# RupertLuo/Valley

Measured on NVIDIA H100. Metric: generated tokens/s (8-frame video requests: ViT-L/14 encode + pool/project + LLaMA prefill + 256 greedy tokens per sequence), higher is better.
Workload: dtype bf16

## Files before the change

### valley_b200/csrc/api.cu

```cuda
#include <cuda_runtime.h>
#include <cuda.h>

#include <algorithm>
#include <atomic>
#include <cmath>
#include <cstdarg>
#include <cstdio>
#include <cstdlib>
#include <cstring>
#include <map>
#include <memory>
#include <mutex>
#include <string>
#include <type_traits>
#include <utility>
#include <vector>

#include "../../include/valley_b200.h"
#include "attention_tc.cuh"
#include "common.cuh"
#include "gemm_tc.cuh"
#include "simt_kernels.cuh"
#include "decode_kernels.cuh"
#include "decode_mega.cuh"
// ... 967 lines not shown
    GemmParams p = {};
    p.M = T * NP; p.N = 2 * H; p.K = H; p.out = KV; p.ldo = 2 * H; p.bias = w.in_b + H;
    TRY(launch_gemm<EPI_BIAS>(c, pick_bn_m(c, p.N, p.M), Xp, H, w.in_w + (size_t)H * H, H, p, st));
    p = {};
    p.M = NP; p.N = H; p.K = H; p.out = Q; p.ldo = H; p.bias = w.in_b;
    TRY(launch_gemm<EPI_BIAS>(c, pick_bn_m(c, p.N, p.M), Xlast, H, w.in_w, H, p, st));
    TRY(launch(c, delta_attention_kernel, {dim3(NP), dim3(nhead * 32), 0, st}, Q, KV, att, T, NP, H, nhead));
    p = {};
    p.M = NP; p.N = H; p.K = H; p.out = X1; p.ldo = H; p.bias = w.out_b; p.residual = Xlast; p.ldr = H;
    TRY(launch_gemm<EPI_BIAS_RES_STATS>(c, pick_bn_m(c, p.N, p.M), att, H, w.out_w, H, p, st));
    TRY(launch(c, layernorm_rows_kernel, {dim3(NP), dim3(256), 0, st}, X1, w.n1_g, w.n1_b, X1, H, 1e-5f));
    p = {};
    p.M = NP; p.N = w.ffn; p.K = H; p.out = F1; p.ldo = w.ffn; p.bias = w.l1_b;
    TRY(launch_gemm<EPI_BIAS>(c, pick_bn_m(c, p.N, p.M), X1, H, w.l1_w, H, p, st));
    TRY(launch(c, relu_inplace_kernel, {dim3(c->num_sms), dim3(256), 0, st}, F1, (long long)NP * w.ffn / 8));
    p = {};
    p.M = NP; p.N = H; p.K = w.ffn; p.out = X2; p.ldo = H; p.bias = w.l2_b; p.residual = X1; p.ldr = H;
    TRY(launch_gemm<EPI_BIAS_RES_STATS>(c, pick_bn_m(c, p.N, p.M), F1, w.ffn, w.l2_w, w.ffn, p, st));
    TRY(launch(c, layernorm_rows_kernel, {dim3(NP), dim3(256), 0, st}, X2, w.n2_g, w.n2_b, X2, H, 1e-5f));
    TRY(launch(c, delta_finish_kernel, two_per_sm, P, X2, vis, T, tokens, H));
  }
  return VLY_OK;
}

extern "C" int vly_pool_project(vly_ctx* c, const void* feats, int n_videos, int T, void* vis_rows, void* stream) {
  if (!c || !feats || !vis_rows || n_videos <= 0 || T <= 0) return fail(VLY_ERR_INVALID, "vly_pool_project: bad argument");
  std::lock_guard<std::mutex> lk(c->mu);
  if (!c->finalized || !c->proj_w) return fail(VLY_ERR_STATE, "vly_pool_project: mm_projector not loaded");
  CK(cudaSetDevice(c->cfg.device));
  cudaStream_t st = (cudaStream_t)stream;
  const vly_config& g = c->cfg;
  const int D = g.vit_hidden, tokens = (g.vit_image / g.vit_patch) * (g.vit_image / g.vit_patch) + 1;
  const int rows = tokens - 1 + T;
  if (g.patch_pooling_method == VLY_POOL_MAX || g.patch_pooling_method == VLY_POOL_TEMPORAL_TRANSFORMER)
    return pool_project_after(c, (const bf16*)feats, n_videos, T, (bf16*)vis_rows, st);
  TRY(ensure(c->w_pool, (size_t)n_videos * rows * D * 2));
  if (g.patch_pooling_method == VLY_POOL_TEMPORAL_IMPORTANCE) {
    if (!c->pool_U) return fail(VLY_ERR_STATE, "vly_pool_project: model.pooling_layer.weight not loaded");
    TRY(ensure(c->w_score, (size_t)n_videos * T * 4));
    TRY(launch(c, importance_score_kernel, {dim3(T, n_videos), dim3(256), 0, st}, (const bf16*)feats, c->pool_U, (float*)c->w_score.p, T,
               tokens, D));
    TRY(launch(c, weighted_pool_kernel, {dim3(c->num_sms * 4), dim3(256), 0, st}, (const bf16*)feats, (const float*)c->w_score.p,
               (bf16*)c->w_pool.p, n_videos, T, tokens, D));
  } else {
    TRY(launch(c, temporal_pool_kernel, {dim3(c->num_sms * 4), dim3(256), 0, st}, (const bf16*)feats, (bf16*)c->w_pool.p, n_videos, T,
               tokens, D));
  }
  GemmParams p = {};
  p.M = n_videos * rows; p.N = g.hidden_size; p.K = D;
  p.out = vis_rows; p.ldo = g.hidden_size; p.bias = c->proj_b;
  return launch_gemm<EPI_BIAS>(c, pick_bn(p.N), (bf16*)c->w_pool.p, D, c->proj_w, D, p, st);
}

extern "C" int vly_embed_splice(vly_ctx* c, const int64_t* ids, const int32_t* src_map, const int32_t* img_idx, const void* vis_rows,
                                int rows_per_img, int B, int S, void* out, void* stream) {
  if (!c || !ids || !out || B <= 0 || S <= 0) return fail(VLY_ERR_INVALID, "vly_embed_splice: bad argument");
  if (src_map && (!img_idx || !vis_rows)) return fail(VLY_ERR_INVALID, "vly_embed_splice: src_map given without img_idx / vis_rows");
  std::lock_guard<std::mutex> lk(c->mu);
  if (!c->finalized || !c->has_llm) return fail(VLY_ERR_STATE, "vly_embed_splice: LLM weights not loaded");
  CK(cudaSetDevice(c->cfg.device));
  return launch(c, embed_splice_kernel, {dim3(B * S), dim3(128), 0, (cudaStream_t)stream}, (const long long*)ids, src_map, img_idx, c->embed,
                (const bf16*)vis_rows, rows_per_img, (bf16*)out, nullptr, 0, S, c->cfg.hidden_size, c->cfg.vocab_size);
}

static void mega_smem_layout(const vly_config& g, int bmax, size_t* x_bytes, size_t* misc) {
  const bool tc = bmax > 1;
  const int kmax = g.intermediate_size > g.hidden_size ? g.intermediate_size : g.hidden_size;
  const size_t xs_stride_b = tc ? (size_t)(((kmax * 2 + 127) & ~127) + MegaCfg::PAD_TC) : (size_t)kmax * 2;
  *x_bytes = ((size_t)bmax * xs_stride_b + 127) & ~size_t(127);
  const int nv = (tc ? MegaCfg::ROWS_TC : MegaCfg::ROWS) * bmax;
  *misc = (2 * MegaCfg::MAX_STAGES + 2 * MegaCfg::RED_SLOTS + 2) * 8 + (size_t)MegaCfg::RED_SLOTS * 16 * nv * 4 + (3 + 16) * bmax * 4 + 256;
}
static const size_t kMegaSmem = 226 * 1024;
static const int kMegaDbgCounters = 1024 * 8;

struct DecodeSettings {
  int stage_kb = 0;
  int rows = 0;
  int inflight_kb = 100;
  int stages = 0;
  int inflight = 0;
  int attn_ikeys = 0;
  int l2_hint = 1;
  bool dbg = false;
};
static DecodeSettings read_decode_settings() {
  auto num = [](const char* name, int unset) {
    const char* v = getenv(name);
    return v ? atoi(v) : unset;
  };
  DecodeSettings s;
  s.stage_kb = num("VLY_MEGA_STAGE_KB", 0);
  s.rows = num("VLY_MEGA_ROWS", 0);
  s.inflight_kb = num("VLY_MEGA_INFLIGHT_KB", 100);
  s.stages = num("VLY_MEGA_STAGES", 0);
  s.inflight = num("VLY_MEGA_INFLIGHT", 0);
  const int ik = num("VLY_ATTN_IKEYS", 0);
  s.attn_ikeys = (ik >= 16 && ik <= 256 && ik % 16 == 0) ? ik : 0;
  const char* hint = getenv("VLY_MEGA_L2_HINT");
  s.l2_hint = (hint && *hint) ? atoi(hint) != 0 : 1;
  s.dbg = getenv("VLY_MEGA_DBG") != nullptr;
  return s;
}

static void pick_phase_geometry(const DecodeSettings& s, int bmax, size_t ring_budget, int N, int K, int num_sms, int* rows_out,
                                int* kc_out) {
  const bool tc = bmax > 1;
  const int max_rows = tc ? MegaCfg::ROWS_TC : MegaCfg::ROWS;
  const int pad = tc ? MegaCfg::PAD_TC : 0, gran = tc ? 64 : 8;
  size_t target = s.stage_kb > 0 ? (size_t)s.stage_kb * 1024 : (tc ? 33 * 1024 + 512 : 41 * 1024);
  if (target > ring_budget / 2) target = ring_budget / 2;
  if (target < 8 * 1024) target = 8 * 1024;
  auto kc_for = [&](int rows) {
    const int cap = (int)((target / rows - pad) / 2);
    const int ns = cdiv(K, cap > gran ? cap : gran);
    int kc = cdiv(cdiv(K, ns), gran) * gran;
    return kc > K ? cdiv(K, gran) * gran : kc;
  };
  int rows = max_rows;
  if (s.rows > 0) rows = s.rows > max_rows ? max_rows : s.rows;
  else {
    if (kc_for(rows) * 2 < 3072 && K * 2 >= 3072) rows = max_rows / 2;
    if (rows == max_rows && !tc) {
      const long long load_full = (long long)cdiv(cdiv(N, max_rows), num_sms) * max_rows;
      const long long load_half = (long long)cdiv(cdiv(N, max_rows / 2), num_sms) * (max_rows / 2);
      if (load_half * 100 < load_full * 97) rows = max_rows / 2;
    }
  }
  *rows_out = rows;
  *kc_out = kc_for(rows);
}

static int plan_decode_mega(vly_ctx* c, vly_kv* kv, const DecodeSettings& s) {
  const vly_config& g = c->cfg;
  const int B = kv->B, H = g.hidden_size, nH = g.num_attention_heads, I = g.intermediate_size, V = g.vocab_size;
  const int bmax = bmax_of(B);
  const int pad = bmax > 1 ? MegaCfg::PAD_TC : 0;
  size_t x_bytes, misc;
  mega_smem_layout(g, bmax, &x_bytes, &misc);
  const size_t ring_budget = kMegaSmem > x_bytes + misc ? kMegaSmem - x_bytes - misc : 0;
  std::vector<PhaseDesc> ph;
  int stage_bytes = 0;
  auto add = [&](PhaseDesc d) {
    d.rows = d.kc = 0;
    if (d.type != PH_ATTN) {
      pick_phase_geometry(s, bmax, ring_budget, d.N, d.K, c->num_sms, &d.rows, &d.kc);
      const int sb = d.rows * (d.kc * 2 + pad);
      if (sb > stage_bytes) stage_bytes = sb;
    }
    ph.push_back(d);
  };
  for (int l = 0; l < g.num_hidden_layers; ++l) {
    const LlamaLayerW& w = c->layers[l];
    PhaseDesc d = {};
    d.layer = l; d.kcache = kv->k_layer(l); d.vcache = kv->v_layer(l);
    d.type = PH_QKV; d.N = 3 * H; d.K = H; d.W = w.wqkv; d.x_in = kv->x; d.out = kv->q; add(d);
    d.type = PH_ATTN; d.N = 0; d.K = 0; d.W = nullptr; d.x_in = nullptr; d.out = kv->attn; add(d);
    d.type = PH_OPROJ; d.N = H; d.K = H; d.W = w.wo; d.x_in = kv->attn; d.out = kv->x; add(d);
    d.type = PH_GATEUP; d.N = 2 * I; d.K = H; d.W = w.wgu; d.x_in = kv->x; d.out = kv->hb; add(d);
    d.type = PH_DOWN; d.N = H; d.K = I; d.W = w.wdown; d.x_in = kv->hb; d.out = kv->x; add(d);
  }
  {
    PhaseDesc d = {};
    d.type = PH_LOGITS; d.N = V; d.K = H; d.W = c->lm_head; d.x_in = kv->x; d.out = nullptr; add(d);
  }
  stage_bytes = (stage_bytes + 127) & ~127;
  for (PhaseDesc& q : ph) {
    if (q.type == PH_ATTN) continue;
    const int sb = q.rows * (q.kc * 2 + pad);
    q.inflight = (s.inflight_kb * 1024 + sb / 2) / sb;
    if (q.inflight < 2) q.inflight = 2;
  }
  int n_stages = (int)(((long long)kMegaSmem - (long long)x_bytes - (long long)misc) / (long long)stage_bytes);
  if (n_stages > MegaCfg::MAX_STAGES) n_stages = MegaCfg::MAX_STAGES;
  const int cap = s.stages > 0 ? s.stages : 4;
  if (n_stages > cap) n_stages = cap;
  if (n_stages < 2)
    return fail(VLY_ERR_INVALID, "vly_kv_create: activations (B=%d, K=%d) leave no room for the weight ring (%d stages, at least 2 needed)",
                B, std::max(I, H), n_stages);
  if (s.dbg) {
    fprintf(stderr, "[vly] decode ring: B=%d x=%zu B, ring budget %zu B, slot %d B, %d slots fit, %d used;", B, x_bytes, ring_budget,
            stage_bytes, (int)(ring_budget / stage_bytes), n_stages);
    for (int i = 0; i < 5 && i < (int)ph.size(); ++i)
      if (ph[i].type != PH_ATTN) fprintf(stderr, " type%d N=%d K=%d rows=%d kc=%d inflight=%d;", ph[i].type, ph[i].N, ph[i].K, ph[i].rows, ph[i].kc, ph[i].inflight);
    fprintf(stderr, " logits rows=%d kc=%d\n", ph.back().rows, ph.back().kc);
    TRY(kv->dbg.alloc(kMegaDbgCounters * sizeof(long long)));
  }
  TRY(kv->d_phases.alloc(ph.size() * sizeof(PhaseDesc)));
  CK(cudaMemcpy(kv->d_phases, ph.data(), ph.size() * sizeof(PhaseDesc), cudaMemcpyHostToDevice));

  StepParams& p = kv->mega;
  p = {};
  p.phases = kv->d_phases; p.n_phases = (int)ph.size();
  p.B = B; p.H = H; p.nH = nH; p.Smax = kv->Smax; p.V = V;
  p.Kmax = std::max(I, H);
  p.eps = g.rms_norm_eps; p.scale_log2e = 0.08838834764831845f * 1.4426950408889634f;
  p.rope = c->rope; p.seq_len = kv->d_len; p.step = kv->d_step; p.embed = c->embed; p.tokens_in = kv->cur_tokens;
  p.x = kv->x; p.q = kv->q; p.attn = kv->attn;
  p.part_o = kv->part_o; p.part_ml = kv->part_ml; p.attn_counters = kv->counters; p.nsplit = kv->nsplit;
  p.key_bits = kv->key_bits; p.mask_words = kv->mask_words();
  p.logits = kv->logits; p.part_val = kv->part_val; p.part_idx = kv->part_idx;
  p.next_tokens = kv->cur_tokens; p.out_tokens = kv->gen_tokens; p.out_stride = kv->Smax;
  p.sample = kv->d_sample;
  p.grid_counter = kv->counters + (size_t)B * nH + 1;
  p.grid_epoch = p.grid_counter + 1;
  p.n_grid_syncs = p.n_phases + 1;
  p.attn_ikeys = s.attn_ikeys;
  p.n_stages = n_stages;
  p.stage_bytes = stage_bytes;
  p.n_inflight = s.inflight > 0 ? s.inflight : n_stages;
  if (p.n_inflight > n_stages) p.n_inflight = n_stages;
  p.l2_hint = s.l2_hint;
  p.dbg = kv->dbg;
  kv->mega_smem = (size_t)n_stages * stage_bytes + x_bytes + misc;
  return VLY_OK;
}

extern "C" int vly_kv_create(vly_ctx* c, int batch, int max_seq, vly_kv** out) {
  if (!c || !out || batch <= 0 || max_seq <= 0) return fail(VLY_ERR_INVALID, "vly_kv_create: bad argument");
  if (!c->finalized || !c->has_llm) return fail(VLY_ERR_STATE, "vly_kv_create: LLM weights not finalised");
  if (max_seq > c->cfg.max_position_embeddings) return fail(VLY_ERR_INVALID, "vly_kv_create: max_seq %d > max_position_embeddings %d", max_seq, c->cfg.max_position_embeddings);
  CK(cudaSetDevice(c->cfg.device));
  const vly_config& g = c->cfg;
  auto kv = std::make_unique<vly_kv>();
  kv->ctx = c;
  kv->B = batch;
  kv->Smax = (max_seq + 127) / 128 * 128;
  const int H = g.hidden_size, nH = g.num_attention_heads, I = g.intermediate_size, V = g.vocab_size, L = g.num_hidden_layers;
  const size_t cache_elems = (size_t)L * kv->layer_stride();
  TRY(kv->cache.alloc(cache_elems * 2));
  CK(cudaMemset(kv->cache, 0, cache_elems * 2));
  kv->nsplit = kv->Smax / MegaCfg::ATTN_KEYS_MIN;
  TRY(kv->d_len.alloc(8));
  TRY(kv->h_len.alloc(sizeof(int), true));
  CK(cudaEventCreateWithFlags(&kv->len_event, cudaEventDisableTiming));
  kv->d_step = kv->d_len + 1;
  CK(cudaMemset(kv->d_len, 0, 8));
  const size_t act_rows = batch < 8 ? 8 : batch;
  TRY(kv->x.alloc(act_rows * H * 2));
  TRY(kv->q.alloc(act_rows * H * 2));
  TRY(kv->attn.alloc(act_rows * H * 2));
  TRY(kv->hb.alloc(act_rows * I * 2));
  CK(cudaMemset(kv->x, 0, act_rows * H * 2));
  CK(cudaMemset(kv->attn, 0, act_rows * H * 2));
  CK(cudaMemset(kv->hb, 0, act_rows * I * 2));
  TRY(kv->part_o.alloc((size_t)batch * nH * kv->nsplit * 128 * 4));
  TRY(kv->part_ml.alloc((size_t)batch * nH * kv->nsplit * sizeof(float2)));
  TRY(kv->counters.alloc(((size_t)batch * nH + 4) * 4));
  CK(cudaMemset(kv->counters, 0, ((size_t)batch * nH + 4) * 4));
  TRY(kv->part_val.alloc((size_t)batch * c->num_sms * 4));
  TRY(kv->part_idx.alloc((size_t)batch * c->num_sms * 4));
  TRY(kv->logits.alloc((size_t)batch * V * 4));
  TRY(kv->cur_tokens.alloc((size_t)batch * 8));
  TRY(kv->gen_tokens.alloc((size_t)batch * kv->Smax * 8));
  TRY(kv->d_sample.alloc(sizeof(SampleState)));
  {
    const SampleState s0 = {};
    CK(cudaMemcpy(kv->d_sample, &s0, sizeof(s0), cudaMemcpyHostToDevice));
  }
  TRY(kv->key_bits.alloc((size_t)batch * kv->mask_words() * 4));
  CK(cudaMemset(kv->key_bits, 0xff, (size_t)batch * kv->mask_words() * 4));
  if (batch <= 4) TRY(plan_decode_mega(c, kv.get(), read_decode_settings()));
  *out = kv.release();
  return VLY_OK;
}

extern "C" int vly_kv_decode_kernel(vly_kv* kv, char* name, int cap) {
  if (!kv || !name || cap <= 0) return fail(VLY_ERR_INVALID, "vly_kv_decode_kernel: bad argument");
  if (kv->B <= 4) snprintf(name, (size_t)cap, "decode_step_kernel<%d>", bmax_of(kv->B));
  else snprintf(name, (size_t)cap, "per-op TMA-ring decode kernels");
  return VLY_OK;
}

extern "C" void vly_kv_destroy(vly_kv* kv) {
  if (!kv) return;
  cudaSetDevice(kv->ctx->cfg.device);
  delete kv;
}

extern "C" int vly_kv_seq_len(vly_kv* kv, int* out) {
  if (!kv || !out) return fail(VLY_ERR_INVALID, "null");
  TRY(sync_len(kv));
  *out = kv->host_len;
  return VLY_OK;
}

extern "C" int vly_kv_reset(vly_kv* kv, void* stream) {
  if (!kv) return fail(VLY_ERR_INVALID, "null");
  CK(cudaSetDevice(kv->ctx->cfg.device));
  kv->host_len = 0;
  kv->len_dirty = false;
  CK(cudaMemsetAsync(kv->d_len, 0, 8, (cudaStream_t)stream));
  if (kv->masked) {
    CK(cudaMemsetAsync(kv->key_bits, 0xff, (size_t)kv->B * kv->mask_words() * 4, (cudaStream_t)stream));
    kv->masked = false;
// ... 753 lines not shown
```

### valley_b200/csrc/common.cuh

```cuda
#pragma once
#include <cuda_runtime.h>
#include <cuda_bf16.h>
#include <cuda_fp16.h>
#include <cuda.h>
#include <stdint.h>

#define VLY_DEVINL __device__ __forceinline__

namespace vly {

VLY_DEVINL uint32_t smem_u32(const void* p) { return static_cast<uint32_t>(__cvta_generic_to_shared(p)); }

VLY_DEVINL uint32_t pack_bf16x2(float lo, float hi) {
  __nv_bfloat162 v = __floats2bfloat162_rn(lo, hi);
  return *reinterpret_cast<uint32_t*>(&v);
}
VLY_DEVINL float bf16_lo(uint32_t v) { return __uint_as_float(v << 16); }
VLY_DEVINL float bf16_hi(uint32_t v) { return __uint_as_float(v & 0xffff0000u); }
VLY_DEVINL float bf16_round(float x) { return __bfloat162float(__float2bfloat16_rn(x)); }

VLY_DEVINL void mbar_init(uint64_t* bar, uint32_t count) {
  asm volatile("mbarrier.init.shared::cta.b64 [%0], %1;\n" ::"r"(smem_u32(bar)), "r"(count));
}
VLY_DEVINL void fence_barrier_init() { asm volatile("fence.mbarrier_init.release.cluster;\n" ::: "memory"); }

VLY_DEVINL void mbar_expect_tx(uint64_t* bar, uint32_t bytes) {
  asm volatile("mbarrier.arrive.expect_tx.shared::cta.b64 _, [%0], %1;\n" ::"r"(smem_u32(bar)), "r"(bytes) : "memory");
}
VLY_DEVINL void mbar_arrive(uint64_t* bar) {
  asm volatile("mbarrier.arrive.shared::cta.b64 _, [%0];\n" ::"r"(smem_u32(bar)) : "memory");
}
VLY_DEVINL bool mbar_try_wait(uint64_t* bar, uint32_t parity) {
  uint32_t ok;
  asm volatile(
      "{\n\t.reg .pred P;\n\t"
      "mbarrier.try_wait.parity.shared::cta.b64 P, [%1], %2;\n\t"
      "selp.b32 %0, 1, 0, P;\n\t}\n"
      : "=r"(ok)
      : "r"(smem_u32(bar)), "r"(parity)
      : "memory");
  return ok != 0;
}
VLY_DEVINL void mbar_wait(uint64_t* bar, uint32_t parity) {
  while (!mbar_try_wait(bar, parity)) {
  }
}

VLY_DEVINL void tma_prefetch_desc(const CUtensorMap* m) {
  asm volatile("prefetch.tensormap [%0];\n" ::"l"(reinterpret_cast<uint64_t>(m)) : "memory");
}
VLY_DEVINL void tma_load_2d(void* smem_dst, const CUtensorMap* m, uint64_t* bar, int c0, int c1) {
  asm volatile(
      "cp.async.bulk.tensor.2d.shared::cluster.global.mbarrier::complete_tx::bytes [%0], [%1, {%3, %4}], [%2];\n" ::"r"(
          smem_u32(smem_dst)),
      "l"(reinterpret_cast<uint64_t>(m)), "r"(smem_u32(bar)), "r"(c0), "r"(c1)
      : "memory");
}
VLY_DEVINL void tma_load_3d(void* smem_dst, const CUtensorMap* m, uint64_t* bar, int c0, int c1, int c2) {
  asm volatile(
      "cp.async.bulk.tensor.3d.shared::cluster.global.mbarrier::complete_tx::bytes [%0], [%1, {%3, %4, %5}], [%2];\n" ::"r"(
          smem_u32(smem_dst)),
      "l"(reinterpret_cast<uint64_t>(m)), "r"(smem_u32(bar)), "r"(c0), "r"(c1), "r"(c2)
      : "memory");
}

VLY_DEVINL void bulk_load_1d(void* smem_dst, const void* gsrc, uint32_t bytes, uint64_t* bar) {
  asm volatile("cp.async.bulk.shared::cluster.global.mbarrier::complete_tx::bytes [%0], [%1], %2, [%3];\n" ::"r"(smem_u32(smem_dst)),
               "l"(gsrc), "r"(bytes), "r"(smem_u32(bar))
               : "memory");
}
VLY_DEVINL void bulk_load_1d_hint(void* smem_dst, const void* gsrc, uint32_t bytes, uint64_t* bar, uint64_t policy) {
  asm volatile("cp.async.bulk.shared::cluster.global.mbarrier::complete_tx::bytes.L2::cache_hint [%0], [%1], %2, [%3], %4;\n" ::"r"(
                   smem_u32(smem_dst)),
               "l"(gsrc), "r"(bytes), "r"(smem_u32(bar)), "l"(policy)
               : "memory");
}
VLY_DEVINL uint64_t l2_policy_evict_first() {
  uint64_t p;
  asm volatile("createpolicy.fractional.L2::evict_first.b64 %0, 1.0;\n" : "=l"(p));
  return p;
}
VLY_DEVINL void pdl_wait() { asm volatile("griddepcontrol.wait;\n" ::: "memory"); }
VLY_DEVINL void pdl_launch_dependents() { asm volatile("griddepcontrol.launch_dependents;\n" ::: "memory"); }

VLY_DEVINL uint64_t make_smem_desc_sw128(uint32_t smem_addr, uint32_t lbo_bytes, uint32_t sbo_bytes) {
  uint64_t d = 0;
  d |= uint64_t((smem_addr >> 4) & 0x3FFF);
  d |= uint64_t((lbo_bytes >> 4) & 0x3FFF) << 16;
  d |= uint64_t((sbo_bytes >> 4) & 0x3FFF) << 32;
  d |= uint64_t(1) << 62;
  return d;
}

VLY_DEVINL float fast_exp2(float x) {
  float y;
  asm("ex2.approx.ftz.f32 %0, %1;" : "=f"(y) : "f"(x));
  return y;
}

VLY_DEVINL float warp_sum(float v) {
#pragma unroll
  for (int o = 16; o > 0; o >>= 1) v += __shfl_xor_sync(0xffffffffu, v, o);
  return v;
}
VLY_DEVINL float warp_max(float v) {
#pragma unroll
  for (int o = 16; o > 0; o >>= 1) v = fmaxf(v, __shfl_xor_sync(0xffffffffu, v, o));
  return v;
}
VLY_DEVINL void warp_argmax(float& v, int& i) {
#pragma unroll
  for (int o = 16; o > 0; o >>= 1) {
    const float ov = __shfl_xor_sync(0xffffffffu, v, o);
    const int oi = __shfl_xor_sync(0xffffffffu, i, o);
    if (ov > v || (ov == v && oi < i)) { v = ov; i = oi; }
  }
}

}
```

### valley_b200/csrc/decode_mega.cuh

```cuda
#pragma once
#include "common.cuh"
#include "simt_kernels.cuh"
#include "decode_kernels.cuh"
#include "sampling.cuh"

namespace vly {

enum PhaseType : int { PH_QKV = 0, PH_ATTN = 1, PH_OPROJ = 2, PH_GATEUP = 3, PH_DOWN = 4, PH_LOGITS = 5 };

struct PhaseDesc {
  int type, N, K, layer;
  int rows, kc;
  int inflight;
  const __nv_bfloat16* W;
  const __nv_bfloat16* x_in;
  __nv_bfloat16* out;
  __nv_bfloat16* kcache;
  __nv_bfloat16* vcache;
};

struct StepParams {
  const PhaseDesc* phases;
  int n_phases;
  int B, H, nH, Smax, V, Kmax;
  float eps, scale_log2e;
  const float2* rope;
  int* seq_len;
  int* step;
  const __nv_bfloat16* embed;
  const long long* tokens_in;
  __nv_bfloat16* x;
  const __nv_bfloat16* q;
  __nv_bfloat16* attn;
  float* part_o;
  float2* part_ml;
  unsigned int* attn_counters;
  int nsplit;
  const uint32_t* key_bits;
  int mask_words;
  float* logits;
  float* part_val;
  int* part_idx;
  long long* next_tokens;
  long long* out_tokens;
  int out_stride;
  SampleState* sample;
  unsigned int* grid_counter;
  unsigned int* grid_epoch;
  int n_grid_syncs;
  int attn_ikeys;
  int n_stages;
  int stage_bytes;
  int n_inflight;
  int l2_hint;
  long long* dbg;
  int select;
};

struct MegaCfg {
  static constexpr int ROWS = 4;
  static constexpr int ROWS_TC = 8;
  static constexpr int PAD_TC = 64;
  static constexpr int CONSUMERS = 512, THREADS = 576;
  static constexpr int RED_SLOTS = 4;
  static constexpr int MAX_STAGES = 8;
  static constexpr int ATTN_KEYS_MIN = 16;
};

VLY_DEVINL uint4 ldcg_v4(const void* p) {
  uint4 r;
  asm volatile("ld.global.cg.v4.u32 {%0, %1, %2, %3}, [%4];\n" : "=r"(r.x), "=r"(r.y), "=r"(r.z), "=r"(r.w) : "l"(p) : "memory");
  return r;
}
VLY_DEVINL float ldcg_bf16(const __nv_bfloat16* p) {
  unsigned short v;
  asm volatile("ld.global.cg.u16 %0, [%1];\n" : "=h"(v) : "l"(p) : "memory");
  return __uint_as_float((uint32_t)v << 16);
}
VLY_DEVINL void mma_m16n8k16_bf16(float (&d)[4], uint32_t a0, uint32_t a1, uint32_t a2, uint32_t a3, uint32_t b0, uint32_t b1) {
  asm volatile("mma.sync.aligned.m16n8k16.row.col.f32.bf16.bf16.f32 {%0,%1,%2,%3}, {%4,%5,%6,%7}, {%8,%9}, {%0,%1,%2,%3};\n"
               : "+f"(d[0]), "+f"(d[1]), "+f"(d[2]), "+f"(d[3])
               : "r"(a0), "r"(a1), "r"(a2), "r"(a3), "r"(b0), "r"(b1));
}

VLY_DEVINL uint32_t ld_acquire_u32(const unsigned int* p) {
  uint32_t v;
  asm volatile("ld.acquire.gpu.global.u32 %0, [%1];\n" : "=r"(v) : "l"(p) : "memory");
  return v;
}
VLY_DEVINL void fence_proxy_async_global() { asm volatile("fence.proxy.async.global;\n" ::: "memory"); }

VLY_DEVINL void grid_sync_consumers(unsigned int* counter, unsigned int target, int ct) {
  asm volatile("bar.sync 2, 544;" ::: "memory");
  if (ct == 0) {
    asm volatile("red.release.gpu.global.add.u32 [%0], 1;\n" ::"l"(counter) : "memory");
    while ((int)(ld_acquire_u32(counter) - target) < 0) {
    }
  }
  asm volatile("bar.sync 2, 544;" ::: "memory");
}

VLY_DEVINL void mega_attention_phase(const StepParams& p, const PhaseDesc& d, const int cw, const int lane, const int pos) {
  const int len = pos + 1;
  const int n_warps = 16 * (int)gridDim.x;
  int ikeys = p.attn_ikeys;
  if (ikeys == 0) {
    if (p.B * p.nH * ((len + 15) >> 4) <= n_warps) ikeys = 16;
    else
      for (ikeys = 32; ikeys < 256; ikeys += 16)
        if (p.B * p.nH * ((len + ikeys - 1) / ikeys) <= n_warps + n_warps / 20) break;
  }
  const int n_act = (len + ikeys - 1) / ikeys;
  const int items = p.B * p.nH * n_act;
  const int hl = lane & 15, hw = lane >> 4;
  for (int it = cw * gridDim.x + blockIdx.x; it < items; it += gridDim.x * 16) {
    const int split = it % n_act, bh = it / n_act;
    const int b = bh / p.nH, h = bh - b * p.nH;
    const int k0 = split * ikeys, nk = min(len - k0, ikeys);
    const __nv_bfloat16* kb = d.kcache + ((size_t)bh * p.Smax + k0) * 128 + hl * 8;
    const __nv_bfloat16* vb = d.vcache + ((size_t)bh * p.Smax + k0) * 128 + hl * 8;
    const uint32_t* kbw = p.key_bits + (size_t)b * p.mask_words;
    float qf[8];
    {
      const uint4 w = ldcg_v4(p.q + (size_t)b * p.H + h * 128 + hl * 8);
      qf[0] = bf16_lo(w.x); qf[1] = bf16_hi(w.x); qf[2] = bf16_lo(w.y); qf[3] = bf16_hi(w.y);
      qf[4] = bf16_lo(w.z); qf[5] = bf16_hi(w.z); qf[6] = bf16_lo(w.w); qf[7] = bf16_hi(w.w);
    }
    float m_run = -INFINITY, l_run = 0.f;
    float o[8] = {0.f, 0.f, 0.f, 0.f, 0.f, 0.f, 0.f, 0.f};
#pragma unroll 1
    for (int kk0 = 0; kk0 < nk; kk0 += 16) {
      const uint32_t kbits = __ldg(kbw + ((k0 + kk0) >> 5)) >> ((k0 + kk0) & 31);
      uint4 kw[8], vw[8];
#pragma unroll
      for (int j = 0; j < 8; ++j) {
        const int key = kk0 + 2 * j + hw;
        const bool ok = key < nk;
        kw[j] = ok ? ldcg_v4(kb + (size_t)key * 128) : make_uint4(0, 0, 0, 0);
        vw[j] = ok ? ldcg_v4(vb + (size_t)key * 128) : make_uint4(0, 0, 0, 0);
      }
      float sc[8];
#pragma unroll
      for (int j = 0; j < 8; ++j) {
        const uint4 w = kw[j];
        sc[j] = qf[0] * bf16_lo(w.x) + qf[1] * bf16_hi(w.x) + qf[2] * bf16_lo(w.y) + qf[3] * bf16_hi(w.y) +
                qf[4] * bf16_lo(w.z) + qf[5] * bf16_hi(w.z) + qf[6] * bf16_lo(w.w) + qf[7] * bf16_hi(w.w);
      }

#pragma unroll
      for (int off = 8, n = 4; off >= 2; off >>= 1, n >>= 1) {
        const bool up = (hl & off) != 0;
#pragma unroll
        for (int i = 0; i < 4; ++i) {
          if (i < n) {
            const float send = up ? sc[i] : sc[i + n];
            const float keep = up ? sc[i + n] : sc[i];
            sc[i] = keep + __shfl_xor_sync(0xffffffffu, send, off);
          }
        }
      }
      sc[0] += __shfl_xor_sync(0xffffffffu, sc[0], 1);
      const int my_key = kk0 + 2 * (hl >> 1) + hw;
      const bool valid = my_key < nk && ((kbits >> (my_key - kk0)) & 1u);
      const float s_my = valid ? sc[0] * p.scale_log2e : -INFINITY;
      float mx = s_my;
      mx = fmaxf(mx, __shfl_xor_sync(0xffffffffu, mx, 2));
// ... 126 lines not shown
      const float ov = __shfl_xor_sync(kMask, bv, o);
      const int oi = __shfl_xor_sync(kMask, bi, o);
      if (ov > bv || (ov == bv && oi < bi)) { bv = ov; bi = oi; }
    }
    if (lane < BMAX && lane < p.B && bv > bestv[lane]) {
      bestv[lane] = bv;
      besti[lane] = bi;
    }
  } else {
    const float mine = t * rstd_s[b];
    const float other = __shfl_xor_sync(kMask, mine, BMAX);
    if ((r & 1) == 0 && ok && n + 1 < d.N) {
      float x0 = mine, x1 = other;
      if (d.type == PH_GATEUP) {
        const float gte = bf16_round(x0), up = bf16_round(x1);
        d.out[(size_t)b * (d.N >> 1) + (n >> 1)] = __float2bfloat16_rn(bf16_round(gte / (1.f + __expf(-gte))) * up);
      } else {
        const int which = n / p.H, nh = n - which * p.H, head = nh >> 7, cidx = nh & 127;
        if (which < 2) {
          const float a = x0 * pre0 - x1 * pre1, c2 = x1 * pre0 + x0 * pre1;
          x0 = a;
          x1 = c2;
        }
        __nv_bfloat16* dst;
        if (which == 0) dst = d.out + (size_t)b * p.H + nh;
        else dst = ((which == 1) ? d.kcache : d.vcache) + (((size_t)b * p.nH + head) * p.Smax + pos) * 128 + cidx;
        *reinterpret_cast<uint32_t*>(dst) = pack_bf16x2(x0, x1);
      }
    }
  }
}

VLY_DEVINL void mega_finish_step(const StepParams& p, const int cw, const int lane, const int ct) {
  if (cw < p.B) {
    const int b = cw;
    float bv = -INFINITY;
    int bi = 0x7fffffff;
    for (int g = lane; g < (int)gridDim.x; g += 32) {
      const float v = __ldcg(p.part_val + (size_t)b * gridDim.x + g);
      const int i = __ldcg(p.part_idx + (size_t)b * gridDim.x + g);
      if (v > bv || (v == bv && i < bi)) { bv = v; bi = i; }
    }
    warp_argmax(bv, bi);
    if (lane == 0) {
      const long long tok = p.select ? sample_finish_row(p.sample, b, bi) : bi;
      p.next_tokens[b] = tok;
      if (p.out_tokens != nullptr) p.out_tokens[(size_t)b * p.out_stride + *p.step] = tok;
    }
  }
  asm volatile("bar.sync 7, 512;" ::: "memory");
  if (ct == 0) {
    *p.step += 1;
    *p.seq_len += 1;
    *p.grid_epoch += 1;
    if (p.select) sample_close_step(p.sample, p.B, true);
    else p.sample->steps_valid += 1;
  }
}

template <int BMAX>
__global__ void __launch_bounds__(576, 1) decode_step_kernel(const StepParams p) {
  using M = MegaCfg;
  constexpr bool kTC = BMAX > 1;
  constexpr int ROWS = kTC ? M::ROWS_TC : M::ROWS;
  constexpr int NV = ROWS * BMAX;
  constexpr int PAD = kTC ? M::PAD_TC : 0;
  extern __shared__ uint8_t msm_raw[];
  uint8_t* msm = msm_raw + ((128u - (smem_u32(msm_raw) & 127u)) & 127u);
  uint8_t* ring = msm;
  __nv_bfloat16* xs = reinterpret_cast<__nv_bfloat16*>(ring + (size_t)p.n_stages * p.stage_bytes);
  const int xs_stride = kTC ? (((p.Kmax * 2 + 127) & ~127) + PAD) / 2 : p.Kmax;
  const size_t xs_bytes = ((size_t)BMAX * xs_stride * 2 + 127) & ~size_t(127);
  uint8_t* tail = reinterpret_cast<uint8_t*>(xs) + xs_bytes;
  uint64_t* full_bar = reinterpret_cast<uint64_t*>(tail);
  uint64_t* empty_bar = full_bar + M::MAX_STAGES;
  uint64_t* red_full = empty_bar + M::MAX_STAGES;
  uint64_t* red_empty = red_full + M::RED_SLOTS;
  uint64_t* x_bar = red_empty + M::RED_SLOTS;
  float* red = reinterpret_cast<float*>(x_bar + 2);
  float* rstd_s = red + M::RED_SLOTS * 16 * NV;
  float* bestv = rstd_s + BMAX;
  int* besti = reinterpret_cast<int*>(bestv + BMAX);
  float* wred = reinterpret_cast<float*>(besti + BMAX);

  const int tid = threadIdx.x, warp = tid >> 5, lane = tid & 31;
  if (p.sample->all_done) return;
  if (tid == 0) {
    for (int i = 0; i < p.n_stages; ++i) {
      mbar_init(&full_bar[i], 1);
      mbar_init(&empty_bar[i], 16);
    }
    for (int i = 0; i < M::RED_SLOTS; ++i) {
      mbar_init(&red_full[i], 16);
      mbar_init(&red_empty[i], 1);
    }
    mbar_init(x_bar, 1);
    fence_barrier_init();
  }
  __syncthreads();

  if (warp == 0) {
    if (lane == 0) {
      int st = 0;
      uint32_t ph = 0;
      int wst = 0, issued = 0, confirmed = 0;
      uint32_t wph = 0;
      long long* dbg_p = p.dbg != nullptr ? p.dbg + (size_t)blockIdx.x * 32 : nullptr;
      if (dbg_p != nullptr)
        for (int i = 26; i < 32; ++i) dbg_p[i] = 0;
      const bool hint = p.l2_hint != 0;
      const uint64_t pol_stream = l2_policy_evict_first();
      for (int pi = 0; pi < p.n_phases; ++pi) {
        const PhaseDesc d = p.phases[pi];
        if (d.type == PH_ATTN) continue;
        const int rows_u = d.rows, KCp = d.kc;
        const int row_stride = KCp * 2 + PAD;
        const int n_groups = (d.N + rows_u - 1) / rows_u;
        const int n_slices = (d.K + KCp - 1) / KCp;
        const int infl = min(d.inflight, p.n_inflight);
        long long t_blocked = 0;
        for (int g = blockIdx.x; g < n_groups; g += gridDim.x) {
          const int n0 = g * rows_u;
          const int rows = min(rows_u, d.N - n0);
          for (int s = 0; s < n_slices; ++s) {
            const int kc = min(KCp, d.K - s * KCp);
            const long long t_w = dbg_p != nullptr ? clock64() : 0;
            mbar_wait(&empty_bar[st], ph ^ 1);
            while (issued - confirmed >= infl) {
              mbar_wait(&full_bar[wst], wph);
              if (++wst == p.n_stages) { wst = 0; wph ^= 1; }
              ++confirmed;
            }
            if (dbg_p != nullptr) t_blocked += clock64() - t_w;
            ++issued;
            mbar_expect_tx(&full_bar[st], (uint32_t)rows * kc * 2);
            uint8_t* dst = ring + (size_t)st * p.stage_bytes;
            const __nv_bfloat16* src = d.W + (size_t)n0 * d.K + (size_t)s * KCp;
            if (PAD == 0 && kc == d.K) {
              if (hint) bulk_load_1d_hint(dst, src, (uint32_t)rows * kc * 2, &full_bar[st], pol_stream);
              else bulk_load_1d(dst, src, (uint32_t)rows * kc * 2, &full_bar[st]);
            } else if (hint) {
              for (int r = 0; r < rows; ++r)
                bulk_load_1d_hint(dst + r * row_stride, src + (size_t)r * d.K, (uint32_t)kc * 2, &full_bar[st], pol_stream);
            } else {
              for (int r = 0; r < rows; ++r) bulk_load_1d(dst + r * row_stride, src + (size_t)r * d.K, (uint32_t)kc * 2, &full_bar[st]);
            }
            if (++st == p.n_stages) { st = 0; ph ^= 1; }
          }
        }
        if (dbg_p != nullptr) dbg_p[26 + d.type] += t_blocked;
      }
    }
    return;
  }

  const bool is_fin = (warp == 17);
  const int ct = tid - 32;
  const int cw = warp - 1;
  const int pos = *p.seq_len;
  const bool samp_on = p.select && p.sample->enabled != 0;
  const float samp_it = p.sample->inv_temp;
  const uint32_t samp_k0 = p.sample->seed_lo, samp_k1 = p.sample->seed_hi;
  unsigned int sync_no = 0;
  const unsigned int sync_base = *p.grid_epoch * (unsigned int)p.n_grid_syncs * gridDim.x;
  long long t_sync = 0, t_stage = 0, t_loop = 0, t_attn = 0, t0 = clock64();
  long long* dbg_o = (p.dbg != nullptr && ct == 0) ? p.dbg + (size_t)blockIdx.x * 32 : nullptr;
  if (dbg_o != nullptr)
    for (int i = 8; i < 26; ++i) dbg_o[i] = 0;
  {
    if (!is_fin) {
      const int chunks = p.B * (p.H >> 3);
      for (int i = blockIdx.x * M::CONSUMERS + ct; i < chunks; i += gridDim.x * M::CONSUMERS) {
        const int b = i / (p.H >> 3), c = i % (p.H >> 3);
        long long id = p.tokens_in[b];
        id = id < 0 ? 0 : (id >= p.V ? p.V - 1 : id);
        *reinterpret_cast<uint4*>(p.x + (size_t)b * p.H + c * 8) = *reinterpret_cast<const uint4*>(p.embed + (size_t)id * p.H + c * 8);
      }
    } else if (lane < BMAX) {
      bestv[lane] = -INFINITY;
      besti[lane] = 0;
    }
    grid_sync_consumers(p.grid_counter, sync_base + (++sync_no) * gridDim.x, ct);
    t_sync += clock64() - t0;
  }

  int st = 0;
  uint32_t ph = 0, xph = 0;
  unsigned int unit_no = 0;
  for (int pi = 0; pi < p.n_phases; ++pi) {
    const PhaseDesc d = p.phases[pi];
    t0 = clock64();
    if (d.type == PH_ATTN) {
      if (!is_fin) mega_attention_phase(p, d, cw, lane, pos);
      t_attn += clock64() - t0;
      if (dbg_o != nullptr) dbg_o[8 + 3 * PH_ATTN + 1] += clock64() - t0;
    } else {
      const bool norm = (d.type == PH_QKV || d.type == PH_GATEUP || d.type == PH_LOGITS);
      const int rows_u = d.rows, KCp = d.kc;
      const int row_stride = KCp * 2 + PAD;
      if (!is_fin) {
        if (ct == 0) {
          fence_proxy_async_global();
          mbar_expect_tx(x_bar, (uint32_t)p.B * d.K * 2);
          for (int b = 0; b < p.B; ++b) bulk_load_1d(xs + (size_t)b * xs_stride, d.x_in + (size_t)b * d.K, (uint32_t)d.K * 2, x_bar);
        }
        mbar_wait(x_bar, xph);
        if (norm) {
          float sq[BMAX];
#pragma unroll
          for (int b = 0; b < BMAX; ++b) sq[b] = 0.f;
          const int chunks = d.K >> 3;
          for (int c = ct; c < chunks; c += M::CONSUMERS) {
#pragma unroll
            for (int b = 0; b < BMAX; ++b) {
              if (b < p.B) {
                const uint4 w = *reinterpret_cast<const uint4*>(xs + (size_t)b * xs_stride + c * 8);
                const uint32_t ww[4] = {w.x, w.y, w.z, w.w};
#pragma unroll
                for (int i = 0; i < 4; ++i) {
                  const float a = bf16_lo(ww[i]), bb = bf16_hi(ww[i]);
                  sq[b] += a * a + bb * bb;
                }
              }
            }
          }
#pragma unroll
          for (int b = 0; b < BMAX; ++b) {
            const float v = warp_sum(sq[b]);
            if (lane == 0) wred[cw * BMAX + b] = v;
          }
        }
      }
      xph ^= 1;
      if (norm) {
        asm volatile("bar.sync 2, 544;" ::: "memory");
        if (!is_fin && ct < BMAX) {
          float t = 0.f;
          for (int w = 0; w < 16; ++w) t += wred[w * BMAX + ct];
          rstd_s[ct] = rsqrtf(t / d.K + p.eps);
        }
        asm volatile("bar.sync 2, 544;" ::: "memory");
      }
      t_stage += clock64() - t0;
      if (dbg_o != nullptr) dbg_o[8 + 3 * d.type] += clock64() - t0;
      t0 = clock64();
      const int n_groups = (d.N + rows_u - 1) / rows_u;
      const int n_slices = (d.K + KCp - 1) / KCp;
      if (!is_fin) {
        for (int g = blockIdx.x; g < n_groups; g += gridDim.x, ++unit_no) {
          const int n0 = g * rows_u;
          const int rows = min(rows_u, d.N - n0);
          const int slot = unit_no & (M::RED_SLOTS - 1);
          const uint32_t round = (unit_no / M::RED_SLOTS) & 1;
          if constexpr (kTC) {
            const int gq = lane >> 2, tq = lane & 3;
            float dacc[4] = {0.f, 0.f, 0.f, 0.f}, dacc1[4] = {0.f, 0.f, 0.f, 0.f};
            const bool w_ok = gq < rows, x_ok = gq < p.B;
            for (int s = 0; s < n_slices; ++s) {
              const int kc = min(KCp, d.K - s * KCp);
              mbar_wait(&full_bar[st], ph);
              const uint8_t* wrow = ring + (size_t)st * p.stage_bytes + gq * row_stride;
              const __nv_bfloat16* xrow = xs + (size_t)gq * xs_stride + (size_t)s * KCp;
              const int nblk = kc >> 5, bpw = (nblk + 15) >> 4;
              const int kb0 = cw * bpw, kb1 = min(kb0 + bpw, nblk);
#pragma unroll 4
              for (int kb = kb0; kb < kb1; ++kb) {
                const int k = kb << 5;
                uint4 wb = make_uint4(0, 0, 0, 0), xa = make_uint4(0, 0, 0, 0);
                if (w_ok) wb = *reinterpret_cast<const uint4*>(wrow + (k + tq * 8) * 2);
                if (x_ok) xa = *reinterpret_cast<const uint4*>(xrow + k + tq * 8);
                mma_m16n8k16_bf16(dacc, xa.x, 0u, xa.y, 0u, wb.x, wb.y);
                mma_m16n8k16_bf16(dacc1, xa.z, 0u, xa.w, 0u, wb.z, wb.w);
              }
              __syncwarp();
              if (lane == 0) mbar_arrive(&empty_bar[st]);
              if (++st == p.n_stages) { st = 0; ph ^= 1; }
            }
            dacc[0] += dacc1[0];
            dacc[1] += dacc1[1];
            mbar_wait(&red_empty[slot], round ^ 1);
            if (gq < BMAX) {
              float* rp = red + (slot * 16 + cw) * NV;
              rp[(2 * tq) * BMAX + gq] = dacc[0];
              rp[(2 * tq + 1) * BMAX + gq] = dacc[1];
            }
            __syncwarp();
            if (lane == 0) mbar_arrive(&red_full[slot]);
            continue;
          }
          float acc[NV];
#pragma unroll
          for (int i = 0; i < NV; ++i) acc[i] = 0.f;
          for (int s = 0; s < n_slices; ++s) {
            const int kc = min(KCp, d.K - s * KCp);
            mbar_wait(&full_bar[st], ph);
            for (int c8 = ct * 8; c8 < kc; c8 += M::CONSUMERS * 8) {
              const uint8_t* src = ring + (size_t)st * p.stage_bytes + c8 * 2;
              float xf[BMAX][8];
#pragma unroll
              for (int b = 0; b < BMAX; ++b) {
                const uint4 xv = *reinterpret_cast<const uint4*>(xs + (size_t)b * xs_stride + (size_t)s * KCp + c8);
                xf[b][0] = bf16_lo(xv.x); xf[b][1] = bf16_hi(xv.x); xf[b][2] = bf16_lo(xv.y); xf[b][3] = bf16_hi(xv.y);
                xf[b][4] = bf16_lo(xv.z); xf[b][5] = bf16_hi(xv.z); xf[b][6] = bf16_lo(xv.w); xf[b][7] = bf16_hi(xv.w);
              }
#pragma unroll
              for (int r = 0; r < ROWS; ++r) {
                if (r < rows) {
                  const uint4 wv = *reinterpret_cast<const uint4*>(src + r * row_stride);
                  const float wf[8] = {bf16_lo(wv.x), bf16_hi(wv.x), bf16_lo(wv.y), bf16_hi(wv.y),
                                       bf16_lo(wv.z), bf16_hi(wv.z), bf16_lo(wv.w), bf16_hi(wv.w)};
#pragma unroll
                  for (int b = 0; b < BMAX; ++b)
#pragma unroll
                    for (int e = 0; e < 8; ++e) acc[r * BMAX + b] = fmaf(wf[e], xf[b][e], acc[r * BMAX + b]);
                }
              }
            }
            __syncwarp();
            if (lane == 0) mbar_arrive(&empty_bar[st]);
            if (++st == p.n_stages) { st = 0; ph ^= 1; }
          }
          warp_reduce_scatter<NV>(acc, lane);
          mbar_wait(&red_empty[slot], round ^ 1);
          if ((lane & (32 / NV - 1)) == 0) red[(slot * 16 + cw) * NV + lane / (32 / NV)] = acc[0];
          __syncwarp();
          if (lane == 0) mbar_arrive(&red_full[slot]);
        }
      } else {
        for (int g = blockIdx.x; g < n_groups; g += gridDim.x, ++unit_no) {
          const int n0 = g * rows_u;
          const int slot = unit_no & (M::RED_SLOTS - 1);
          const uint32_t round = (unit_no / M::RED_SLOTS) & 1;
          const int r = lane / BMAX, b = lane % BMAX, n = n0 + r;
          const bool ok = lane < NV && r < rows_u && b < p.B && n < d.N;
          float pre0 = 0.f, pre1 = 0.f;
          mega_epilogue_prefetch(p, d, ok, b, n, pos, pre0, pre1);
          mbar_wait(&red_full[slot], round);
          float t = 0.f;
          if (lane < NV) {
#pragma unroll
            for (int w = 0; w < 16; ++w) t += red[(slot * 16 + w) * NV + lane];
          }
          __syncwarp();
          if (lane == 0) mbar_arrive(&red_empty[slot]);
          if (lane < NV)
            mega_unit_epilogue<BMAX, NV>(p, d, lane, t, ok, r, b, n, pre0, pre1, pos, rstd_s, bestv, besti, samp_on, samp_it, samp_k0, samp_k1);
        }
      }
      t_loop += clock64() - t0;
      if (dbg_o != nullptr) dbg_o[8 + 3 * d.type + 1] += clock64() - t0;
    }
    t0 = clock64();
    if (pi == p.n_phases - 1 && is_fin && lane < p.B) {
      p.part_val[(size_t)lane * gridDim.x + blockIdx.x] = bestv[lane];
      p.part_idx[(size_t)lane * gridDim.x + blockIdx.x] = besti[lane];
    }
    grid_sync_consumers(p.grid_counter, sync_base + (++sync_no) * gridDim.x, ct);
    t_sync += clock64() - t0;
    if (dbg_o != nullptr) dbg_o[8 + 3 * d.type + 2] += clock64() - t0;
  }
  if (dbg_o != nullptr) {
    dbg_o[0] = t_sync; dbg_o[1] = t_stage; dbg_o[2] = t_loop; dbg_o[3] = t_attn; dbg_o[4] = 0;
  }

  if (blockIdx.x == 0 && !is_fin) mega_finish_step(p, cw, lane, ct);
}

}
```

Before: 387.8.

## Prefetch upcoming decode weights into L2 while consumers sit at grid syncs

Restructures the megakernel's weight producer loop around a cursor over all phases/groups/slices and adds a second lookahead cursor. A shared state word marks when the consumers are in their x-staging or grid-sync window, and during that time the producer issues cp.async.bulk.prefetch.L2 for up to a configurable number of bytes (default 96 KB) ahead of the current load position. Waits become try_wait polling so prefetches can be interleaved. The intent is to hide the HBM latency bubble at phase boundaries. The cost is extra L2 traffic, possible interference with the evict_first streaming policy, and more producer-side control overhead.

```diff
diff --git a/valley_b200/csrc/api.cu b/valley_b200/csrc/api.cu
--- a/valley_b200/csrc/api.cu
+++ b/valley_b200/csrc/api.cu
@@ -1073,6 +1073,7 @@
   int inflight = 0;
   int attn_ikeys = 0;
   int l2_hint = 1;
+  int l2_ahead_kb = 96;
   bool dbg = false;
 };
 static DecodeSettings read_decode_settings() {
@@ -1090,6 +1091,7 @@
   s.attn_ikeys = (ik >= 16 && ik <= 256 && ik % 16 == 0) ? ik : 0;
   const char* hint = getenv("VLY_MEGA_L2_HINT");
   s.l2_hint = (hint && *hint) ? atoi(hint) != 0 : 1;
+  s.l2_ahead_kb = std::min(std::max(num("VLY_MEGA_L2_AHEAD_KB", 96), 0), 256);
   s.dbg = getenv("VLY_MEGA_DBG") != nullptr;
   return s;
 }
@@ -1202,6 +1204,7 @@
   p.n_inflight = s.inflight > 0 ? s.inflight : n_stages;
   if (p.n_inflight > n_stages) p.n_inflight = n_stages;
   p.l2_hint = s.l2_hint;
+  p.l2_ahead = s.l2_ahead_kb * 1024;
   p.dbg = kv->dbg;
   kv->mega_smem = (size_t)n_stages * stage_bytes + x_bytes + misc;
   return VLY_OK;
diff --git a/valley_b200/csrc/common.cuh b/valley_b200/csrc/common.cuh
--- a/valley_b200/csrc/common.cuh
+++ b/valley_b200/csrc/common.cuh
@@ -80,6 +80,9 @@
   asm volatile("createpolicy.fractional.L2::evict_first.b64 %0, 1.0;\n" : "=l"(p));
   return p;
 }
+VLY_DEVINL void bulk_prefetch_l2(const void* gsrc, uint32_t bytes) {
+  asm volatile("cp.async.bulk.prefetch.L2.global [%0], %1;\n" ::"l"(gsrc), "r"(bytes) : "memory");
+}
 VLY_DEVINL void pdl_wait() { asm volatile("griddepcontrol.wait;\n" ::: "memory"); }
 VLY_DEVINL void pdl_launch_dependents() { asm volatile("griddepcontrol.launch_dependents;\n" ::: "memory"); }
 
diff --git a/valley_b200/csrc/decode_mega.cuh b/valley_b200/csrc/decode_mega.cuh
--- a/valley_b200/csrc/decode_mega.cuh
+++ b/valley_b200/csrc/decode_mega.cuh
@@ -53,6 +53,7 @@
   int stage_bytes;
   int n_inflight;
   int l2_hint;
+  int l2_ahead;
   long long* dbg;
   int select;
 };
@@ -82,6 +83,39 @@
                : "+f"(d[0]), "+f"(d[1]), "+f"(d[2]), "+f"(d[3])
                : "r"(a0), "r"(a1), "r"(a2), "r"(a3), "r"(b0), "r"(b1));
 }
+
+struct MegaCursor {
+  int pi, g, s;
+  long long off;
+  const __nv_bfloat16* W;
+  int type, N, K, rows_u, kcp, n_groups, n_slices, infl;
+
+  VLY_DEVINL void enter(const StepParams& p, int pi_) {
+    for (pi = pi_; pi < p.n_phases; ++pi) {
+      const PhaseDesc d = p.phases[pi];
+      if (d.type == PH_ATTN) continue;
+      n_groups = (d.N + d.rows - 1) / d.rows;
+      if ((int)blockIdx.x >= n_groups) continue;
+      W = d.W; type = d.type; N = d.N; K = d.K; rows_u = d.rows; kcp = d.kc;
+      n_slices = (d.K + d.kc - 1) / d.kc;
+      infl = min(d.inflight, p.n_inflight);
+      break;
+    }
+    g = blockIdx.x;
+    s = 0;
+  }
+  VLY_DEVINL bool done(const StepParams& p) const { return pi >= p.n_phases; }
+  VLY_DEVINL int rows() const { return min(rows_u, N - g * rows_u); }
+  VLY_DEVINL int kc() const { return min(kcp, K - s * kcp); }
+  VLY_DEVINL const __nv_bfloat16* src() const { return W + (size_t)g * rows_u * K + (size_t)s * kcp; }
+  VLY_DEVINL void next(const StepParams& p) {
+    off += (long long)rows() * kc() * 2;
+    if (++s < n_slices) return;
+    s = 0;
+    g += gridDim.x;
+    if (g >= n_groups) enter(p, pi + 1);
+  }
+};
 
 VLY_DEVINL uint32_t ld_acquire_u32(const unsigned int* p) {
   uint32_t v;
@@ -374,6 +408,7 @@
   float* bestv = rstd_s + BMAX;
   int* besti = reinterpret_cast<int*>(bestv + BMAX);
   float* wred = reinterpret_cast<float*>(besti + BMAX);
+  volatile int* cstate = reinterpret_cast<volatile int*>(wred + 16 * BMAX);
 
   const int tid = threadIdx.x, warp = tid >> 5, lane = tid & 31;
   if (p.sample->all_done) return;
@@ -388,6 +423,7 @@
     }
     mbar_init(x_bar, 1);
     fence_barrier_init();
+    *cstate = 0;
   }
   __syncthreads();
 
@@ -398,49 +434,71 @@
       int wst = 0, issued = 0, confirmed = 0;
       uint32_t wph = 0;
       long long* dbg_p = p.dbg != nullptr ? p.dbg + (size_t)blockIdx.x * 32 : nullptr;
-      if (dbg_p != nullptr)
+      if (dbg_p != nullptr) {
         for (int i = 26; i < 32; ++i) dbg_p[i] = 0;
+        for (int i = 5; i < 8; ++i) dbg_p[i] = 0;
+      }
+      long long pf_bytes = 0, t_win = 0;
       const bool hint = p.l2_hint != 0;
       const uint64_t pol_stream = l2_policy_evict_first();
-      for (int pi = 0; pi < p.n_phases; ++pi) {
-        const PhaseDesc d = p.phases[pi];
-        if (d.type == PH_ATTN) continue;
-        const int rows_u = d.rows, KCp = d.kc;
-        const int row_stride = KCp * 2 + PAD;
-        const int n_groups = (d.N + rows_u - 1) / rows_u;
-        const int n_slices = (d.K + KCp - 1) / KCp;
-        const int infl = min(d.inflight, p.n_inflight);
-        long long t_blocked = 0;
-        for (int g = blockIdx.x; g < n_groups; g += gridDim.x) {
-          const int n0 = g * rows_u;
-          const int rows = min(rows_u, d.N - n0);
-          for (int s = 0; s < n_slices; ++s) {
-            const int kc = min(KCp, d.K - s * KCp);
-            const long long t_w = dbg_p != nullptr ? clock64() : 0;
-            mbar_wait(&empty_bar[st], ph ^ 1);
-            while (issued - confirmed >= infl) {
-              mbar_wait(&full_bar[wst], wph);
+      MegaCursor fc, pf;
+      fc.off = 0;
+      fc.enter(p, 0);
+      pf = fc;
+      while (!fc.done(p)) {
+        const long long t_w = dbg_p != nullptr ? clock64() : 0;
+        long long t_poll = t_w;
+        bool slot_free = false;
+        for (;;) {
+          if (!slot_free) slot_free = mbar_try_wait(&empty_bar[st], ph ^ 1);
+          if (slot_free) {
+            while (issued - confirmed >= fc.infl && mbar_try_wait(&full_bar[wst], wph)) {
               if (++wst == p.n_stages) { wst = 0; wph ^= 1; }
               ++confirmed;
             }
-            if (dbg_p != nullptr) t_blocked += clock64() - t_w;
-            ++issued;
-            mbar_expect_tx(&full_bar[st], (uint32_t)rows * kc * 2);
-            uint8_t* dst = ring + (size_t)st * p.stage_bytes;
-            const __nv_bfloat16* src = d.W + (size_t)n0 * d.K + (size_t)s * KCp;
-            if (PAD == 0 && kc == d.K) {
-              if (hint) bulk_load_1d_hint(dst, src, (uint32_t)rows * kc * 2, &full_bar[st], pol_stream);
-              else bulk_load_1d(dst, src, (uint32_t)rows * kc * 2, &full_bar[st]);
-            } else if (hint) {
-              for (int r = 0; r < rows; ++r)
-                bulk_load_1d_hint(dst + r * row_stride, src + (size_t)r * d.K, (uint32_t)kc * 2, &full_bar[st], pol_stream);
-            } else {
-              for (int r = 0; r < rows; ++r) bulk_load_1d(dst + r * row_stride, src + (size_t)r * d.K, (uint32_t)kc * 2, &full_bar[st]);
+            if (issued - confirmed < fc.infl) break;
+          }
+          const bool window = (*cstate & 1) == 0;
+          if (dbg_p != nullptr) {
+            const long long t = clock64();
+            if (window) t_win += t - t_poll;
+            t_poll = t;
+          }
+          if (window) {
+            while (!pf.done(p) && pf.off - fc.off < p.l2_ahead) {
+              const int rows = pf.rows(), kc = pf.kc();
+              const __nv_bfloat16* src = pf.src();
+              if (PAD == 0 && kc == pf.K) bulk_prefetch_l2(src, (uint32_t)rows * kc * 2);
+              else
+                for (int r = 0; r < rows; ++r) bulk_prefetch_l2(src + (size_t)r * pf.K, (uint32_t)kc * 2);
+              pf_bytes += (long long)rows * kc * 2;
+              pf.next(p);
             }
-            if (++st == p.n_stages) { st = 0; ph ^= 1; }
-          }
-        }
-        if (dbg_p != nullptr) dbg_p[26 + d.type] += t_blocked;
+          }
+        }
+        if (dbg_p != nullptr) dbg_p[26 + fc.type] += clock64() - t_w;
+        ++issued;
+        const int rows = fc.rows(), kc = fc.kc();
+        const int row_stride = fc.kcp * 2 + PAD;
+        mbar_expect_tx(&full_bar[st], (uint32_t)rows * kc * 2);
+        uint8_t* dst = ring + (size_t)st * p.stage_bytes;
+        const __nv_bfloat16* src = fc.src();
+        if (PAD == 0 && kc == fc.K) {
+          if (hint) bulk_load_1d_hint(dst, src, (uint32_t)rows * kc * 2, &full_bar[st], pol_stream);
+          else bulk_load_1d(dst, src, (uint32_t)rows * kc * 2, &full_bar[st]);
+        } else if (hint) {
+          for (int r = 0; r < rows; ++r)
+            bulk_load_1d_hint(dst + r * row_stride, src + (size_t)r * fc.K, (uint32_t)kc * 2, &full_bar[st], pol_stream);
+        } else {
+          for (int r = 0; r < rows; ++r) bulk_load_1d(dst + r * row_stride, src + (size_t)r * fc.K, (uint32_t)kc * 2, &full_bar[st]);
+        }
+        if (++st == p.n_stages) { st = 0; ph ^= 1; }
+        fc.next(p);
+        if (pf.off < fc.off) pf = fc;
+      }
+      if (dbg_p != nullptr) {
+        dbg_p[5] = pf_bytes;
+        dbg_p[6] = t_win;
       }
     }
     return;
@@ -483,6 +541,7 @@
     const PhaseDesc d = p.phases[pi];
     t0 = clock64();
     if (d.type == PH_ATTN) {
+      if (ct == 0) *cstate = 2 * pi + 1;
       if (!is_fin) mega_attention_phase(p, d, cw, lane, pos);
       t_attn += clock64() - t0;
       if (dbg_o != nullptr) dbg_o[8 + 3 * PH_ATTN + 1] += clock64() - t0;
@@ -538,6 +597,7 @@
       t0 = clock64();
       const int n_groups = (d.N + rows_u - 1) / rows_u;
       const int n_slices = (d.K + KCp - 1) / KCp;
+      if (ct == 0) *cstate = 2 * pi + 1;
       if (!is_fin) {
         for (int g = blockIdx.x; g < n_groups; g += gridDim.x, ++unit_no) {
           const int n0 = g * rows_u;
@@ -648,6 +708,7 @@
       p.part_idx[(size_t)lane * gridDim.x + blockIdx.x] = besti[lane];
     }
     grid_sync_consumers(p.grid_counter, sync_base + (++sync_no) * gridDim.x, ct);
+    if (ct == 0) *cstate = 2 * pi + 2;
     t_sync += clock64() - t0;
     if (dbg_o != nullptr) dbg_o[8 + 3 * d.type + 2] += clock64() - t0;
   }
```

After: 393.5, median of 6. 1.01x the previous value.
